# codeMonkey339/Congestion-control-with-BitTorren

Hardware: AMD Instinct MI355X
Metric: GiB/s device-resident SHA-1 over 512KB chunks; % of HBM-read roofline (higher is better)
Workload: dtype u32; 1 GPU; 4096 x 524288 B chunks per GPU, device-resident (BASELINE config 2); chunks_per_gpu=4096, chunk_bytes=524288, kernel=split_u4_2prod, kernel_requested=auto, streams=1, parallelism=chunk-sharded x1, no collective

## Files before the change

### congestion-control-with-bittorren_amd/csrc/rt_device.hip

```cpp
#include <algorithm>
#include <cctype>
#include <cstdarg>
#include <cstdio>
#include <cstdlib>
#include <cstring>
#include <mutex>
#include <sched.h>
#include <string>
#include <vector>

#include "sha1_runtime_internal.h"

using namespace s1rt;

namespace {
std::string sysfs_line(const char* path) {
    char buf[4096] = {0};
    if (FILE* f = fopen(path, "r")) {
        if (!fgets(buf, sizeof buf, f)) buf[0] = 0;
        fclose(f);
    }
    return buf;
}

// ... 107 lines not shown
    va_end(ap);
    t_err = buf;
    return code;
}

std::string g_probe_err;
Device* g_dev = nullptr;

int device_count() {
    std::call_once(g_once, probe);
    return g_count;
}

int ensure_slots(Device& D, int n) {
    for (int i = 0; i < n && i < kMaxSlots; ++i) {
        Slot& s = D.slot[i];
        if (s.stream) continue;
        HIP_TRY(hipEventCreateWithFlags(&s.done, hipEventDisableTiming));
        HIP_TRY(hipEventCreateWithFlags(&s.copied, hipEventDisableTiming));
        HIP_TRY(hipStreamCreateWithFlags(&s.stream, hipStreamNonBlocking));
    }
    return SHA1CHUNK_OK;
}

int ensure_copy(Device& D) {
    if (!D.copy) HIP_TRY(hipStreamCreateWithFlags(&D.copy, hipStreamNonBlocking));
    return SHA1CHUNK_OK;
}

int get_device(Device** out) {
    if (device_count() <= 0) return fail(SHA1CHUNK_ENODEV, "%s", g_probe_err.c_str());
    if (t_dev < 0 || t_dev >= g_count) return fail(SHA1CHUNK_EINVAL, "bad device %d", t_dev);
    Device& D = g_dev[t_dev];
    HIP_TRY(hipSetDevice(D.id));
    if (!D.ready.load(std::memory_order_acquire)) {
        std::lock_guard<std::mutex> lk(D.mu);
        if (!D.ready.load(std::memory_order_relaxed)) {
            hipDeviceProp_t pr;
            HIP_TRY(hipGetDeviceProperties(&pr, D.id));
            D.cus = pr.multiProcessorCount;
            int rc = ensure_slots(D, 1);
            if (rc) return rc;
            D.ready.store(true, std::memory_order_release);
        }
    }
    *out = &D;
    return SHA1CHUNK_OK;
}

int copies_issued(Slot& s, hipStream_t cs) {
    if (cs == s.stream) return SHA1CHUNK_OK;
    HIP_TRY(hipEventRecord(s.copied, cs));
    HIP_TRY(hipStreamWaitEvent(s.stream, s.copied, 0));
    return SHA1CHUNK_OK;
}

int discard_in_flight(Device& D) {
    for (auto& s : D.slot) {
        if (!s.busy) continue;
        s.busy = false;
        HIP_TRY(hipEventSynchronize(s.done));
    }
    return SHA1CHUNK_OK;
}

int drain_cus_take(Device* D) {
    const int want = static_cast<int>(
        std::max<uint64_t>(1, std::min<uint64_t>({static_cast<uint64_t>(D->cus), 1024, env_u64("SHA1CHUNK_VQ_CUS", 64)})));
    const int budget = static_cast<int>(std::min<uint64_t>(
        static_cast<uint64_t>(D->cus), env_u64("SHA1CHUNK_VQ_CU_BUDGET", static_cast<uint64_t>(D->cus / 2))));
    std::lock_guard<std::mutex> lk(D->drain_mu);
    const int left = budget - D->drain_cus;
    const int take = std::min(want, left);
    if (take < std::min(want, 8)) return 0;
    D->drain_cus += take;
    return take;
}

void drain_cus_give(int dev, int cus) {
    if (dev < 0 || dev >= g_count) return;
    std::lock_guard<std::mutex> lk(g_dev[dev].drain_mu);
    g_dev[dev].drain_cus -= cus;
}
}

extern "C" {

int s1be_device_count(void) {
    const int n = device_count();
    if (n <= 0) fail(SHA1CHUNK_ENODEV, "%s", g_probe_err.c_str());
    return n;
}

int s1be_set_device(int device) {
    const int n = device_count();
    if (n <= 0) return fail(SHA1CHUNK_ENODEV, "%s", g_probe_err.c_str());
    if (device < 0 || device >= n) return fail(SHA1CHUNK_EINVAL, "device %d of %d", device, n);
    t_dev = device;
    return SHA1CHUNK_OK;
}

const char* s1be_last_error(void) { return t_err.c_str(); }

int s1be_device_pci_bus_id(int device, char* buf, size_t len) {
    const int n = device_count();
    if (n <= 0) return fail(SHA1CHUNK_ENODEV, "%s", g_probe_err.c_str());
    if (device < 0 || device >= n) return fail(SHA1CHUNK_EINVAL, "device %d of %d", device, n);
    if (len > static_cast<size_t>(INT32_MAX)) len = INT32_MAX;
    HIP_TRY(hipDeviceGetPCIBusId(buf, static_cast<int>(len), g_dev[device].id));
    return SHA1CHUNK_OK;
}

int s1be_receive_cpus(int device, unsigned slot, void* mask, size_t len, unsigned* domains) {
    const int n = device_count();
    if (n <= 0) return fail(SHA1CHUNK_ENODEV, "%s", g_probe_err.c_str());
    if (device < 0 || device >= n) return fail(SHA1CHUNK_EINVAL, "device %d of %d", device, n);
    const std::vector<cpu_set_t>& dom = receive_domains(g_dev[device].id);
    if (dom.empty()) return fail(SHA1CHUNK_EINVAL, "no CPU of this process's affinity mask found");
    const cpu_set_t& d = dom[slot % dom.size()];
    memset(mask, 0, len);
    memcpy(mask, &d, sizeof d);
    if (domains) *domains = static_cast<unsigned>(dom.size());
    return CPU_COUNT(&d);
}

}
```

### congestion-control-with-bittorren_amd/csrc/sha1_kernels.h

```cpp
#pragma once

#include <hip/hip_runtime.h>
#include <stdint.h>

struct BatchArgs {
    const uint8_t* base;
    const uint64_t* off;
    const uint32_t* len;
    uint32_t ulen;
    uint32_t n;
    const uint32_t* order;
    uint8_t* dig;
    const uint32_t* init_state;
    uint64_t prefix_bytes;
    uint32_t* out_state;
    const uint32_t* plan;
};

hipError_t launch_lane(const BatchArgs& A, hipStream_t st);
hipError_t launch_fused(const BatchArgs& A, hipStream_t st);
bool split_unit_built(int unit_blocks);
hipError_t launch_split(const BatchArgs& A, int unit_blocks, hipStream_t st);
bool split_unit_study_built(int unit_blocks);
hipError_t launch_split_study(const BatchArgs& A, int unit_blocks, hipStream_t st);
uint32_t mixed_grid(uint32_t groups, int cus, uint32_t* hcap);
constexpr uint32_t kBigExact = 4096;
struct BigFix {
    const uint32_t* cnt;
    uint32_t tiles;
    const uint32_t* len;
    const uint32_t* id;
    uint32_t* order;
    uint32_t* sorted_len;
};
hipError_t launch_mixed(const BatchArgs& A, const uint32_t* sorted_len, const BigFix* big, uint32_t* plan, int cus,
                        const int* forced, hipStream_t st);
hipError_t launch_plan_layout(const BatchArgs& A, const uint32_t* sorted_len, const BigFix* big, uint32_t* plan,
                              hipStream_t st);
struct VqDrainArgs {
    const uint8_t* data;
    const uint64_t* off;
    const uint32_t* len;
    const uint8_t* exp;
    const uint32_t* grp;
    const uint32_t* pub;
    const uint32_t* stop;
    uint8_t* alive;
    uint8_t* res;
    uint32_t* done;
    uint32_t* last_done;
    uint8_t* dig;
    uint32_t* claim;
    uint32_t grp_ring;
    uint32_t pad;
    uint64_t idle_ticks;
    uint64_t life_ticks;
};
hipError_t launch_vq_drain(const VqDrainArgs& Q, uint32_t grid, hipStream_t st);

struct PvEntry {
    uint32_t session;
    uint32_t from;
    uint32_t upto;
    uint32_t len;
    uint32_t final;
    uint32_t gen;
    uint32_t pad[2];
};
struct PvArgs {
    const uint8_t* data;
    uint64_t stride;
    const PvEntry* work;
    uint32_t n;
    uint32_t sessions;
    uint32_t* state;
    const uint32_t* expected;
    uint32_t* result;
    uint32_t* done;
    const uint8_t* dummy;
};
hipError_t launch_progress(const PvArgs& P, int depth, hipStream_t st);
hipError_t launch_progress_shared(const PvArgs& P, hipStream_t st);

struct UpdateArgs {
    uint8_t* ctx;
    uint64_t n_contexts;
    const uint32_t* index;
    uint32_t n;
    const uint8_t* base;
    const uint64_t* off;
    const uint32_t* len;
    uint64_t* mid_off;
    uint32_t* mid_len;
    uint32_t* state;
    uint8_t* dig;
};
hipError_t launch_update_init(const UpdateArgs& U, hipStream_t st);
hipError_t launch_update_pre(const UpdateArgs& U, hipStream_t st);
hipError_t launch_update_post(const UpdateArgs& U, hipStream_t st);
hipError_t launch_update_final(const UpdateArgs& U, hipStream_t st);

struct GatherArgs {
    const uint8_t* base;
// ... 33 lines not shown
```

### congestion-control-with-bittorren_amd/csrc/sha1_kernels.hip

```cpp
#include <hip/hip_runtime.h>
#include <stdint.h>

#include <algorithm>
#include <cstdlib>
#include <cstring>

#include "sha1_split.hpp"

#define PLAN_SPLIT4 0.743
#define PLAN_SPLIT8 0.860
#define PLAN_FUSED4T 1.254
#define PLAN_FUSED4S 1.334
#define PLAN_FUSED8T 2.502
#define PLAN_FUSED8S 2.628
#define PLAN_FUSED_SHARE 0.955

__global__ __launch_bounds__(256) void sha1_lane_kernel(BatchArgs A) {
    const uint32_t e = blockIdx.x * blockDim.x + threadIdx.x;
    if (e >= A.n) return;
    const Entry en = fetch_entry(A, e);
    uint32_t h[5];
    load_init(A, en.id, h);
    lane_blocks(A, en, 0, h);
    emit(A, en.id, h);
// ... 777 lines not shown
    if (t < kMaxCand) {
        uint64_t key = t < nref ? (uint64_t)__float_as_uint(cmk[t]) << 32 | t : ~0ull;
#pragma unroll
        for (uint32_t m = 32; m >= 1; m >>= 1) key = min(key, (uint64_t)__shfl_xor(key, m));
        if (lane == 0u) red[wv] = key;
    }
    __syncthreads();
    if (t == 0) {
        ts[5] = __builtin_amdgcn_s_memrealtime();
        cs[5] = __builtin_amdgcn_s_memtime();
        uint64_t key = red[0];
#pragma unroll
        for (uint32_t w = 1; w < kMaxCand / 64; ++w) key = min(key, red[w]);
        uint32_t bi = (uint32_t)key;
        if (cmk[2] <= cmk[bi] * 1.005f) bi = 2;
        plan[0] = cmode[bi];
        plan[1] = cmode[bi] == 1 ? 0u : chead[bi];
        plan[2] = cmode[bi] == 1 ? 0u : cf[bi];
#pragma unroll
        for (int i = 1; i < 6; ++i) plan[7 + i] = static_cast<uint32_t>(ts[i] - ts[0]);
#pragma unroll
        for (int i = 1; i < 6; ++i) plan[13 + i] = static_cast<uint32_t>(cs[i] - cs[0]);
#pragma unroll
        for (int i = 0; i < 3; ++i) plan[20 + i] = static_cast<uint32_t>(sub[i] - cs[0]);
        plan[23] = nrun;
#pragma unroll
        for (int i = 0; i < 3; ++i) plan[24 + i] = static_cast<uint32_t>(bsub[i] - cs[0]);
        plan[27] = simcyc;
    }
}

__device__ __forceinline__ uint64_t splitmix64(uint64_t x) {
    uint64_t z = x + 0x9E3779B97F4A7C15ull;
    z = (z ^ (z >> 30)) * 0xBF58476D1CE4E5B9ull;
    z = (z ^ (z >> 27)) * 0x94D049BB133111EBull;
    return z ^ (z >> 31);
}

__global__ __launch_bounds__(kSynthThreads) void synth_fill_kernel(uint8_t* dst, const uint64_t* off,
                                                         const uint32_t* lens, uint32_t ulen,
                                                         uint64_t first, uint64_t seed) {
    const uint64_t c = blockIdx.x;
    const uint32_t len = lens ? lens[c] : ulen;
    uint8_t* out = dst + (off ? off[c] : c * (uint64_t)ulen);
    const uint64_t key = seed ^ ((first + c) << 24);
    const uint32_t nw = len >> 3;
    uint64_t* o = reinterpret_cast<uint64_t*>(out);
    for (uint32_t w = threadIdx.x; w < nw; w += blockDim.x) o[w] = splitmix64(key ^ (uint64_t)w);
    const uint32_t rem = len & 7u;
    if (rem && threadIdx.x == 0) {
        const uint64_t v = splitmix64(key ^ (uint64_t)nw);
        for (uint32_t b = 0; b < rem; ++b) out[8ull * nw + b] = (uint8_t)(v >> (8 * b));
    }
}

__global__ __launch_bounds__(256) void compare_kernel(const uint8_t* dig, const uint8_t* exp,
                                                      uint32_t n, uint8_t* mismatch) {
    const uint32_t i = blockIdx.x * blockDim.x + threadIdx.x;
    if (i >= n) return;
    uint32_t diff = 0;
#pragma unroll
    for (int b = 0; b < 20; ++b) diff |= (uint32_t)(dig[20ull * i + b] ^ exp[20ull * i + b]);
    mismatch[i] = diff ? 1 : 0;
}

hipError_t launch_lane(const BatchArgs& A, hipStream_t st) {
    if (A.n == 0) return hipSuccess;
    const uint32_t grid = (A.n + 255u) / 256u;
    hipLaunchKernelGGL(sha1_lane_kernel, dim3(grid), dim3(256), 0, st, A);
    return hipGetLastError();
}

hipError_t launch_fused(const BatchArgs& A, hipStream_t st) {
    if (A.n == 0) return hipSuccess;
    hipLaunchKernelGGL(sha1_fused_kernel, dim3((A.n + 255u) / 256u), dim3(256), 0, st, A);
    return hipGetLastError();
}

__attribute__((weak)) bool split_unit_study_built(int) { return false; }
__attribute__((weak)) hipError_t launch_split_study(const BatchArgs&, int, hipStream_t) {
    return hipErrorInvalidValue;
}

bool split_unit_built(int u) { return u == 1 || u == 4 || u == 11 || split_unit_study_built(u); }

hipError_t launch_split(const BatchArgs& A, int unit_blocks, hipStream_t st) {
    if (A.n == 0) return hipSuccess;
    const uint32_t groups = (A.n + 63u) / 64u;
    switch (unit_blocks) {
    case 1: hipLaunchKernelGGL((sha1_split_kernel<1, 1>), dim3(groups), dim3(128), 0, st, A); break;
    case 4:
        hipLaunchKernelGGL((sha1_split_kernel<4, 1, kSplitV<4>, kSplitNProd<4>>), dim3(groups),
                           dim3(64 * (1 + kSplitNProd<4>) + ((kSplitV<4> & kVSkipWave2) ? 64 : 0)), 0,
                           st, A);
        break;
    case 11:
        if (A.off == nullptr && A.order == nullptr)
            hipLaunchKernelGGL((sha1_split_kernel<2, 2, kSplit8V & ~kVCoop, 2>), dim3((groups + 1) / 2), dim3(512),
                               0, st, A);
        else
            hipLaunchKernelGGL((sha1_split_kernel<2, 2, kSplit8V, 2>), dim3((groups + 1) / 2), dim3(512), 0,
                               st, A);
        break;
    default: return launch_split_study(A, unit_blocks, st);
    }
    return hipGetLastError();
}

uint32_t mixed_grid(uint32_t groups, int cus, uint32_t* hcap) {
    *hcap = std::min<uint32_t>(std::min<uint32_t>(groups, 4u * (uint32_t)cus), kPlanMaxH);
    return groups;
}

hipError_t launch_plan_layout(const BatchArgs& A, const uint32_t* sorted_len, const BigFix* big, uint32_t* plan,
                              hipStream_t st) {
    if (A.n == 0) return hipSuccess;
    const uint32_t groups = (A.n + 63u) / 64u;
    const uint32_t words = (groups + 31u) / 32u;
    uint64_t* lay_tb = reinterpret_cast<uint64_t*>(plan + 64);
    uint32_t* lay_bits = reinterpret_cast<uint32_t*>(lay_tb + words);
    uint32_t* lay_blk = lay_bits + words;
    hipLaunchKernelGGL(plan_layout_kernel, dim3(words), dim3(kLayoutThreads), 0, st, A, sorted_len,
                       big ? *big : BigFix{}, lay_tb, lay_bits, lay_blk);
    return hipGetLastError();
}

hipError_t launch_mixed(const BatchArgs& A, const uint32_t* sorted_len, const BigFix* big, uint32_t* plan, int cus,
                        const int* forced, hipStream_t st) {
    if (A.n == 0) return hipSuccess;
    const uint32_t groups = (A.n + 63u) / 64u;
    uint32_t hcap;
    const uint32_t grid = mixed_grid(groups, cus, &hcap);
    const uint32_t words = (groups + 31u) / 32u;
    uint64_t* lay_tb = reinterpret_cast<uint64_t*>(plan + 64);
    uint32_t* lay_bits = reinterpret_cast<uint32_t*>(lay_tb + words);
    const uint32_t* lay_blk = lay_bits + words;
    if (!forced) {
        const hipError_t le = launch_plan_layout(A, sorted_len, big, plan, st);
        if (le != hipSuccess) return le;
    }
    hipLaunchKernelGGL(plan_mixed_kernel, dim3(1), dim3(kPlanThreads), 0, st, A, sorted_len,
                       (uint32_t)cus, hcap, forced ? 1 : 0, forced ? (uint32_t)forced[0] : 0u,
                       forced ? (uint32_t)forced[1] : 0u, forced ? (uint32_t)forced[2] : 0u, plan, lay_tb,
                       lay_bits, lay_blk);
    hipError_t e = hipGetLastError();
    if (e != hipSuccess) return e;
    BatchArgs B = A;
    B.plan = plan;
    const char* disp = getenv("SHA1CHUNK_MIXED_DISPATCH");
    const bool persistent = !(disp && !strcmp(disp, "hw"));
    if (persistent)
        hipLaunchKernelGGL(sha1_mixed_persistent_kernel, dim3((uint32_t)cus), dim3(kMixedThreads), 0, st, B,
                           plan + 3);
    else
        hipLaunchKernelGGL(sha1_mixed_kernel, dim3(grid), dim3(kMixedThreads), 0, st, B);
    return hipGetLastError();
}

hipError_t launch_vq_drain(const VqDrainArgs& Q, uint32_t grid, hipStream_t st) {
    hipLaunchKernelGGL(sha1_vq_drain_kernel, dim3(grid), dim3(kMixedThreads), 0, st, Q);
    return hipGetLastError();
}

hipError_t launch_synth(uint8_t* dst, const uint64_t* off, const uint32_t* lens, uint32_t ulen,
                        uint64_t first, uint64_t count, uint64_t seed, hipStream_t st) {
    if (count == 0) return hipSuccess;
    if (count > kSynthMaxChunks) return hipErrorInvalidValue;
    hipLaunchKernelGGL(synth_fill_kernel, dim3((uint32_t)count), dim3(kSynthThreads), 0, st, dst, off, lens,
                       ulen, first, seed);
    return hipGetLastError();
}

hipError_t launch_compare(const uint8_t* dig, const uint8_t* exp, uint32_t n, uint8_t* mismatch,
                          hipStream_t st) {
    if (n == 0) return hipSuccess;
    hipLaunchKernelGGL(compare_kernel, dim3((n + 255u) / 256u), dim3(256), 0, st, dig, exp, n,
                       mismatch);
    return hipGetLastError();
}

#ifdef SHA1CHUNK_CHECKED
extern "C" __attribute__((visibility("default"))) long long s1be_checked_violations(int reset) {
    int cur = 0, nd = 0;
    if (hipGetDevice(&cur) != hipSuccess || hipGetDeviceCount(&nd) != hipSuccess) return -1;
    long long total = 0;
    for (int d = 0; d < nd; ++d) {
// ... 15 lines not shown
```

### congestion-control-with-bittorren_amd/csrc/sha1_runtime.hip

```cpp
#include <algorithm>
#include <cstdio>
#include <cstdlib>
#include <cstring>
#include <mutex>
#include <numeric>
#include <string>
#include <thread>
#include <vector>

#include "sha1_runtime_internal.h"

using namespace s1rt;

namespace {
int split_unit(size_t n, int cus) {
    if (const char* e = getenv("SHA1CHUNK_SPLIT_UNIT")) return atoi(e);
    const size_t groups = (n + 63) / 64;
    if (groups <= size_t(cus)) return 4;
    if (groups <= size_t(cus) * 2) return 11;
    return 1;
}

hipError_t launch(int kernel, const BatchArgs& A, int cus, hipStream_t st) {
    switch (kernel) {
    case SHA1CHUNK_KERNEL_LANE: return launch_lane(A, st);
    case SHA1CHUNK_KERNEL_FUSED: return launch_fused(A, st);
    case SHA1CHUNK_KERNEL_SPLIT: return launch_split(A, split_unit(A.n, cus), st);
    default: return hipErrorInvalidValue;
    }
}

int check_batch(const BatchArgs& A) {
    if (A.n > 0xffffffffu - 1024u)
        return fail(SHA1CHUNK_EINVAL, "batch of %u chunks: at most 2^32 - 1025 per call", A.n);
    if (A.n > 0 && (reinterpret_cast<uintptr_t>(A.dig) & 3u))
        return fail(SHA1CHUNK_EALIGN, "digest buffer must be 4-byte aligned");
    return SHA1CHUNK_OK;
}
}

namespace s1rt {
int choose_kernel(int kernel, size_t n, int cus) {
    if (kernel != SHA1CHUNK_KERNEL_AUTO) return kernel;
    if (const char* f = getenv("SHA1CHUNK_FORCE_KERNEL")) {
        if (!strcmp(f, "lane")) return SHA1CHUNK_KERNEL_LANE;
        if (!strcmp(f, "fused")) return SHA1CHUNK_KERNEL_FUSED;
        if (!strcmp(f, "split")) return SHA1CHUNK_KERNEL_SPLIT;
    }
    const size_t groups = (n + 63) / 64;
    return groups <= size_t(cus) * 2 ? SHA1CHUNK_KERNEL_SPLIT : SHA1CHUNK_KERNEL_FUSED;
}

int launch_checked(int kernel, const BatchArgs& A, hipStream_t st, int cus) {
    if (kernel < SHA1CHUNK_KERNEL_LANE || kernel > SHA1CHUNK_KERNEL_SPLIT)
        return fail(SHA1CHUNK_EINVAL, "unknown kernel id %d", kernel);
    if (int rc = check_batch(A)) return rc;
    if (kernel == SHA1CHUNK_KERNEL_SPLIT && !split_unit_built(split_unit(A.n, cus)))
        return fail(SHA1CHUNK_EINVAL, "split shape %d is not in this library (A/B shapes: `make ab`)",
                    split_unit(A.n, cus));
    hipError_t e = launch(kernel, A, cus, st);
    if (e != hipSuccess) return fail(SHA1CHUNK_EHIP, "kernel launch: %s", hipGetErrorString(e));
    return SHA1CHUNK_OK;
}

bool use_mixed(size_t n, int cus) {
    if (getenv("SHA1CHUNK_FORCE_KERNEL")) return false;
    const char* e = getenv("SHA1CHUNK_MIXED");
    if (e && !strcmp(e, "0")) return false;
    if (e && !strcmp(e, "all")) return true;
    return (n + 63) / 64 > size_t(cus);
}

int launch_mixed_checked(const BatchArgs& A, const uint32_t* sorted_len, const BigFix* big, uint32_t* plan, int cus,
                         hipStream_t st) {
    if (int rc = check_batch(A)) return rc;
    int forced[3] = {0, 0, 0};
    bool force = false;
    if (const char* e = getenv("SHA1CHUNK_MIXED_PLAN")) {
        uint32_t hcap;
        const uint32_t groups = (A.n + 63u) / 64u;
        (void)mixed_grid(groups, cus, &hcap);
        if (sscanf(e, "%d,%d,%d", &forced[0], &forced[1], &forced[2]) != 3 || forced[0] < 0 ||
            forced[0] > 1 ||
            (forced[0] == 0 && (forced[1] < 0 || ((uint32_t)forced[1] > hcap && (uint32_t)forced[1] != groups) ||
                                (forced[2] != 4 && forced[2] != 8))))
            return fail(SHA1CHUNK_EINVAL,
                        "SHA1CHUNK_MIXED_PLAN=%s: want 0,H,F (0 <= H <= %u or H = %u, F 4|8) or 1,0,0", e,
                        hcap, groups);
        force = true;
    }
    hipError_t e = launch_mixed(A, sorted_len, big, plan, cus, force ? forced : nullptr, st);
    if (e != hipSuccess) return fail(SHA1CHUNK_EHIP, "mixed kernel launch: %s", hipGetErrorString(e));
    if (const char* d = getenv("SHA1CHUNK_MIXED_DEBUG"); d && atoi(d)) {
        uint32_t p[28];
        HIP_TRY(hipMemcpyAsync(p, plan, sizeof p, hipMemcpyDeviceToHost, st));
        HIP_TRY(hipStreamSynchronize(st));
        fprintf(stderr, "sha1chunk mixed plan: n=%u groups=%u cus=%d mode=%u H=%u F=%u\n", A.n,
                (A.n + 63u) / 64u, cus, p[0], p[1], p[2]);
        if (!force && p[12])
// ... 472 lines not shown
```

### congestion-control-with-bittorren_amd/csrc/sha1_runtime_internal.h

```cpp
#pragma once

#include <hip/hip_runtime.h>

#include <algorithm>
#include <atomic>
#include <cstdint>
#include <cstdlib>
#include <ctime>
#include <memory>
#include <mutex>
#include <sched.h>
#include <string>
#include <vector>

#include "../../include/sha1chunk.h"
#include "part_pool.hpp"
#include "sha1_kernels.h"

extern "C" const char* s1be_last_error(void);

namespace s1rt {
using s1host::PartPool;

int fail(int code, const char* fmt, ...) __attribute__((format(printf, 2, 3)));
// ... 13 lines not shown
    const char* e = getenv(name);
    return e ? strtoull(e, nullptr, 10) : dflt;
}

inline int64_t mono_ns() {
    timespec ts;
    clock_gettime(CLOCK_MONOTONIC, &ts);
    return int64_t(ts.tv_sec) * 1000000000 + ts.tv_nsec;
}

struct DevBuf {
    void* p = nullptr;
    size_t cap = 0;
    int ensure(size_t bytes) {
        if (bytes <= cap) return SHA1CHUNK_OK;
        if (p) (void)hipFree(p);
        p = nullptr;
        cap = 0;
        bytes = round_up(std::max(bytes, size_t(1) << 20), size_t(1) << 20);
        if (hipMalloc(&p, bytes) != hipSuccess)
            return fail(SHA1CHUNK_ENOMEM, "hipMalloc(%zu) failed", bytes);
        cap = bytes;
        return SHA1CHUNK_OK;
    }
};

struct PinBuf {
    void* p = nullptr;
    size_t cap = 0;
    int ensure(size_t bytes) {
        if (bytes <= cap) return SHA1CHUNK_OK;
        if (p) (void)hipHostFree(p);
        p = nullptr;
        cap = 0;
        bytes = round_up(std::max(bytes, size_t(1) << 20), size_t(1) << 20);
        if (hipHostMalloc(&p, bytes, hipHostMallocDefault) != hipSuccess)
            return fail(SHA1CHUNK_ENOMEM, "hipHostMalloc(%zu) failed", bytes);
        cap = bytes;
        return SHA1CHUNK_OK;
    }
};

constexpr int kMaxSlots = 8;

struct Slot {
    PinBuf hpin;
    PinBuf hdig;
    DevBuf dmem;
    DevBuf ddig;
    hipStream_t stream = nullptr;
    hipEvent_t done = nullptr;
    hipEvent_t copied = nullptr;
    bool busy = false;
    std::vector<uint32_t> ids;
};

struct Device {
    std::mutex mu;
    std::atomic<bool> ready{false};
    int id = -1;
    int cus = 256;
    Slot slot[kMaxSlots];
    hipStream_t copy = nullptr;
    DevBuf small;
    PinBuf small_pin;
    std::unique_ptr<PartPool> pack;
    std::mutex drain_mu;
    int drain_cus = 0;
};

extern Device* g_dev;
extern std::string g_probe_err;
extern thread_local int t_dev;
int device_count();
int get_device(Device** out);
int ensure_slots(Device& D, int n);
int ensure_copy(Device& D);
int copies_issued(Slot& s, hipStream_t cs);
int discard_in_flight(Device& D);
const cpu_set_t* near_cpus(int id);
const std::vector<cpu_set_t>& receive_domains(int id);
int drain_cus_take(Device* D);
void drain_cus_give(int dev, int cus);

int choose_kernel(int kernel, size_t n, int cus);
int launch_checked(int kernel, const BatchArgs& A, hipStream_t st, int cus = 256);
bool use_mixed(size_t n, int cus);
int launch_mixed_checked(const BatchArgs& A, const uint32_t* sorted_len, const BigFix* big, uint32_t* plan, int cus,
                         hipStream_t st);
bool host_pinned(const void* p);
int pack_threads();

int vq_copy_helpers();
unsigned ring_flags();
int vq_stream_create(hipStream_t* s);
}
```

### congestion-control-with-bittorren_amd/csrc/sha1_split.hpp

```cpp
#ifndef SHA1_SPLIT_HPP
#define SHA1_SPLIT_HPP

#include <hip/hip_runtime.h>
#include <stdint.h>

#include "sha1_device.hpp"
#include "sha1_kernels.h"

using namespace s1;

namespace {

struct Entry {
    uint32_t id;
    const uint8_t* p;
    uint32_t len;
};

#ifdef SHA1CHUNK_CHECKED
__device__ unsigned int g_checked_oob;

__device__ __forceinline__ uint32_t checked_index(uint32_t i, uint32_t n, const char* what) {
    if (i < n) return i;
    if (atomicAdd(&g_checked_oob, 1u) < 8u)
// ... 400 lines not shown
        read_w_group<3>(slot, Wn);
        __builtin_amdgcn_sched_barrier(0);
        RoundsW<R + 40, 80, WK>::run(v, Wc);
    } else {
        constexpr int R = PH != 0 ? 10 : 0;
        if constexpr (jn == 0) split_barrier_or_timed<V>(bw);
        RoundsW<0, R, WK>::run(v, Wc);
        __builtin_amdgcn_sched_barrier(0);
        read_w_group<0>(slot, Wn);
        __builtin_amdgcn_sched_barrier(0);
        RoundsW<R, R + 20, WK>::run(v, Wc);
        __builtin_amdgcn_sched_barrier(0);
        read_w_group<1>(slot, Wn);
        __builtin_amdgcn_sched_barrier(0);
        RoundsW<R + 20, R + 40, WK>::run(v, Wc);
        __builtin_amdgcn_sched_barrier(0);
        read_w_group<2>(slot, Wn);
        __builtin_amdgcn_sched_barrier(0);
        RoundsW<R + 40, R + 60, WK>::run(v, Wc);
        __builtin_amdgcn_sched_barrier(0);
        read_w_group<3>(slot, Wn);
        __builtin_amdgcn_sched_barrier(0);
        RoundsW<R + 60, 80, WK>::run(v, Wc);
    }
    if constexpr (MASK) {
        const bool live = k < T;
#pragma unroll
        for (int i = 0; i < 5; ++i) h[i] = live ? h[i] + v[i] : h[i];
    } else {
#pragma unroll
        for (int i = 0; i < 5; ++i) h[i] += v[i];
    }
}

template <int U, int J, int V, bool MASK, int PH = 0>
struct ConsumeUnits {
    __device__ __forceinline__ static void run(uint32_t k0, uint32_t T, uint32_t (&h)[5],
                                               uint32_t (&Wa)[80], uint32_t (&Wb)[80],
                                               const uint8_t* ring, int lane, uint64_t& bw) {
        if constexpr (J < 2 * U) {
            consume_block<U, J, V, MASK, PH>(k0 + J, T, h, Wa, Wb, ring, lane, bw);
            ConsumeUnits<U, J + 1, V, MASK, PH>::run(k0, T, h, Wb, Wa, ring, lane, bw);
        }
    }
};

template <int U, int V, int PH>
__device__ __forceinline__ void consume_all(const BatchArgs& A, const Entry& en, bool valid, uint32_t T,
                                            uint32_t units, const uint8_t* ring, int lane) {
    uint32_t h[5];
    load_init(A, en.id, h);
    uint32_t Wa[80], Wb[80];
    split_barrier();
    read_w_group<0>(ring + lane * 16, Wa);
    read_w_group<1>(ring + lane * 16, Wa);
    read_w_group<2>(ring + lane * 16, Wa);
    read_w_group<3>(ring + lane * 16, Wa);
    const uint32_t Tmin = __builtin_amdgcn_readfirstlane(wave_min(valid ? T : 0xffffffffu));
    const uint32_t full = (V & kVUnmask) ? min(Tmin, units * U) / (2 * U) * (2 * U) : 0u;
    uint32_t k = 0;
    uint64_t bw = 0;
    const uint64_t t0 = (V & kVProbe) ? __builtin_amdgcn_s_memtime() : 0;
    for (; k < full; k += 2 * U) {
        ConsumeUnits<U, 0, V, false, PH>::run(k, T, h, Wa, Wb, ring, lane, bw);
    }
    for (; k < units * U; k += 2 * U) {
        ConsumeUnits<U, 0, V, true, PH>::run(k, T, h, Wa, Wb, ring, lane, bw);
    }
    if constexpr ((V & kVProbe) != 0) {
        const uint64_t tot = __builtin_amdgcn_s_memtime() - t0;
        if (lane == 0) {
            uint32_t* o = reinterpret_cast<uint32_t*>(A.dig + 20ull * (en.id & ~63u));
            o[0] = (uint32_t)bw;
            o[1] = (uint32_t)(bw >> 32);
            o[2] = (uint32_t)tot;
            o[3] = (uint32_t)(tot >> 32);
            o[4] = units * U;
        }
        return;
    }
    if (valid) emit(A, en.id, h);
}

template <int U, int PAIRS, int V, int NPROD>
__device__ __forceinline__ void split_body(const BatchArgs& A, uint8_t* lds, uint32_t wg) {
    constexpr bool WK = (V & kVWK) != 0;
    static_assert(PAIRS * 2 * U * kWBlockBytes <= 160 * 1024, "LDS");
    static_assert(NPROD == 1 || (PAIRS == 1 && (U == 2 * NPROD || U == NPROD)) ||
                      (PAIRS == 2 && U == NPROD && (V & kVLayout8) != 0),
                  "two producers: one stage (U = 4) or one block (U = 2, 8-wave layout) each per unit");
    int wave = __builtin_amdgcn_readfirstlane(threadIdx.x >> 6);
    if constexpr ((V & kVSimdRole) != 0) {
        static_assert(PAIRS == 1 && NPROD == 2 && U == 2, "SIMD roles: one pair, two producers, 2-block units");
        uint32_t* slots = reinterpret_cast<uint32_t*>(lds);
        const uint32_t hw = __builtin_amdgcn_s_getreg((31u << 11) | (0u << 6) | 4u);
        if ((threadIdx.x & 63u) == 0) slots[1 + wave] = (hw >> 4) & 3u;
        if (threadIdx.x == 0) slots[0] = cu_turn(hw);
        __syncthreads();
        const uint32_t cs = (__builtin_amdgcn_readfirstlane(slots[0]) & 1u) ? 2u : 0u;
        int wc = -1, wi = -1;
        for (int w = 0; w < 4; ++w)
            if (wc < 0 && slots[1 + w] == cs) wc = w;
        if (wc < 0) wc = 0;
        for (int w = 0; w < 4; ++w)
            if (wi < 0 && w != wc && slots[1 + w] == (cs ^ 2u)) wi = w;
        if (wi < 0) wi = wc == 3 ? 2 : 3;
        int rank = 0;
        for (int w = 0; w < wave; ++w) rank += (w != wc && w != wi) ? 1 : 0;
        __syncthreads();
        if (wave == wi) return;
        wave = wave == wc ? 0 : 1 + rank;
    }
    if constexpr ((V & kVSkipWave2) != 0) {
        static_assert(NPROD == 2 && PAIRS == 1, "skip-wave layout is for two producers");
        if (wave == 2) return;
        if (wave > 2) wave -= 1;
    }
    int pair = wave % PAIRS;
    bool producer = wave >= PAIRS;
    uint32_t pidx = producer ? (uint32_t)(wave - PAIRS) / PAIRS : 0u;
    if constexpr ((V & kVLayout8) != 0) {
        static_assert(PAIRS == 2 && NPROD == 2, "8-wave layout: two pairs, two producers each");
        if (wave == 4 || wave == 6) return;
        producer = (wave & 1) != 0;
        pair = producer ? (((wave >> 1) & 1) ^ ((V & kVCross) ? 1 : 0)) : (wave >> 1);
        pidx = producer ? (uint32_t)(wave >> 2) : 0u;
    }
    const int lane = threadIdx.x & 63;
    uint8_t* ring = lds + pair * (2 * U * kWBlockBytes);
    const uint32_t group = wg * PAIRS + (uint32_t)pair;
    const uint32_t e = group * 64u + (uint32_t)lane;
    const bool valid = e < A.n;
    Entry en = fetch_entry(A, valid ? e : fallback_entry(A, group));
    if (!valid) en.len = 0;
    const uint32_t T = valid ? (A.out_state ? (en.len >> 6) : total_blocks(en.len)) : 0u;
    uint32_t Tmax = __builtin_amdgcn_readfirstlane(wave_max(T));
    if constexpr (PAIRS > 1) {
        uint32_t* slots = reinterpret_cast<uint32_t*>(lds);
        if (!producer && lane == 0) slots[pair] = Tmax;
        __syncthreads();
#pragma unroll
        for (int q = 0; q < PAIRS; ++q) Tmax = max(Tmax, slots[q]);
        Tmax = __builtin_amdgcn_readfirstlane(Tmax);
        __syncthreads();
    }
    const uint32_t units = (Tmax + 2 * U - 1) / (2 * U) * 2;

    if (producer) {
        const uint32_t S = bulk_stages(en, valid);
        if constexpr (U == NPROD) {
            const uint32_t K = S * 2u;
            uint32_t B0[16], B1[16];
            uint32_t k = pidx;
            uint64_t pbw = 0;
            uint64_t* const pb = (V & kVProbe) ? &pbw : nullptr;
            const uint64_t pt0 = (V & kVProbe) ? __builtin_amdgcn_s_memtime() : 0;
            if constexpr ((V & kVCoop) != 0) {
                const u32x4u* src[4];
                coop_sources<4>(A, group, (uint32_t)lane, src);
                if (pidx < K) coop4_load(src, pidx, B0);
                if (pidx + NPROD < K) coop4_load(src, pidx + NPROD, B1);
                for (; k + NPROD < K; k += 2 * NPROD) {
                    produce_own_block_coop<U, WK, NPROD>(src, k, K, B0, ring, (uint32_t)lane, pb);
                    produce_own_block_coop<U, WK, NPROD>(src, k + NPROD, K, B1, ring, (uint32_t)lane, pb);
                }
                if (k < K) {
                    produce_own_block_coop<U, WK, NPROD>(src, k, K, B0, ring, (uint32_t)lane, pb);
                    k += NPROD;
// ... 7 lines not shown
                }
                if (k < K) {
                    produce_own_block<U, WK, NPROD>(en, k, K, B0, ring, lane, pb);
                    k += NPROD;
                }
            }
            for (; k < units * U; k += NPROD) {
                uint32_t w[16];
                if (k < T) tail_block_words(en, k, w);
                produce_block<U, WK, NPROD>(k, w, ring, lane, pb);
            }
            if constexpr ((V & kVProbe) != 0) {
                const uint64_t tot = __builtin_amdgcn_s_memtime() - pt0;
                if (lane == 0) {
                    uint32_t* o = reinterpret_cast<uint32_t*>(A.dig + 20ull * (group * 64u + 1u + pidx));
                    o[0] = (uint32_t)pbw;
                    o[1] = (uint32_t)(pbw >> 32);
                    o[2] = (uint32_t)tot;
                    o[3] = (uint32_t)(tot >> 32);
                    o[4] = units * U;
                }
            }
            split_barrier();
            return;
        }
        uint32_t s = pidx;
        if constexpr ((V & kVCoop) != 0) {
            const u32x4u* src[8];
            coop_sources<8>(A, group, (uint32_t)lane, src);
            uint32_t C0[32], C1[32];
            if (pidx < S) coop_load(src, pidx, C0);
            if (pidx + NPROD < S) coop_load(src, pidx + NPROD, C1);
            for (; s + NPROD < S; s += 2 * NPROD) {
                produce_stage_coop<U, WK, NPROD>(src, s, S, C0, ring, (uint32_t)lane);
                produce_stage_coop<U, WK, NPROD>(src, s + NPROD, S, C1, ring, (uint32_t)lane);
            }
            if (s < S) {
                produce_stage_coop<U, WK, NPROD>(src, s, S, C0, ring, (uint32_t)lane);
                s += NPROD;
            }
        } else {
            Stage A0, A1;
            if (pidx < S) load_stage(en.p + 128ull * pidx, A0);
            if (pidx + NPROD < S) load_stage(en.p + 128ull * (pidx + NPROD), A1);
            for (; s + NPROD < S; s += 2 * NPROD) {
                produce_stage<U, WK, NPROD>(en, s, S, A0, ring, lane);
                produce_stage<U, WK, NPROD>(en, s + NPROD, S, A1, ring, lane);
            }
            if (s < S) {
                produce_stage<U, WK, NPROD>(en, s, S, A0, ring, lane);
                s += NPROD;
            }
        }
        for (; 2 * s < units * U; s += NPROD) {
#pragma unroll
            for (int half = 0; half < 2; ++half) {
                const uint32_t k = 2 * s + half;
                uint32_t w[16];
                if (k < T) tail_block_words(en, k, w);
                produce_block<U, WK, NPROD>(k, w, ring, lane);
            }
        }
        split_barrier();
    } else {
        if constexpr ((V & kVPhase2) != 0) {
            if (pair == 1)
                consume_all<U, V, 3>(A, en, valid, T, units, ring, lane);
            else
                consume_all<U, V, 1>(A, en, valid, T, units, ring, lane);
            return;
        }
        if constexpr ((V & kVPhase) != 0) {
            if (pair == 1) {
                consume_all<U, V, 2>(A, en, valid, T, units, ring, lane);
                return;
            }
        }
        consume_all<U, V, 0>(A, en, valid, T, units, ring, lane);
    }
}

constexpr int kSplit8V = kVWK | kVUnmask | kVLayout8 | kVCross | kVCoop;

template <int U, int PAIRS, int V = kSplitV<U>, int NPROD = 1>
__global__ __launch_bounds__((kSplitThreads<PAIRS, V, NPROD>)) void sha1_split_kernel(
    BatchArgs A) {
    __shared__ __attribute__((aligned(16))) uint8_t lds[PAIRS * 2 * U * kWBlockBytes];
    split_body<U, PAIRS, V, NPROD>(A, lds, blockIdx.x);
}


template <typename V>
__device__ __forceinline__ void fused_stage(uint32_t s, uint32_t S, const Entry& en, Stage& cur,
                                            uint32_t (&h)[5]) {
#pragma unroll
    for (int half = 0; half < 2; ++half) {
        uint32_t w[16];
#pragma unroll
        for (int j = 0; j < 16; ++j) w[j] = bswap_fresh(cur.w[16 * half + j]);
        if (half == 1 && s + 2 < S) load_stage<V>(en.p + 128ull * (s + 2), cur);
        compress(h, w);
    }
}

template <typename V>
__device__ __forceinline__ void fused_lane_stages_v(const Entry& en, uint32_t S, uint32_t (&h)[5]) {
    Stage A0, A1;
    if (S > 0) load_stage<V>(en.p, A0);
    if (S > 1) load_stage<V>(en.p + 128, A1);
    uint32_t s = 0;
    for (; s + 1 < S; s += 2) {
        fused_stage<V>(s, S, en, A0, h);
        fused_stage<V>(s + 1, S, en, A1, h);
    }
    if (s < S) fused_stage<V>(s, S, en, A0, h);
}

__device__ __forceinline__ void fused_stage_any(uint32_t s, uint32_t S, const Entry& en, RawSpan<32>& cur,
                                                uint32_t (&h)[5]) {
    const uint32_t sh = static_cast<uint32_t>(reinterpret_cast<uintptr_t>(en.p) & 3u);
    uint32_t w[16];
    shift_raw<32, 0, 16>(cur, sh, w);
#pragma unroll
    for (int j = 0; j < 16; ++j) w[j] = bswap_fresh(w[j]);
    compress(h, w);
    shift_raw<32, 16, 16>(cur, sh, w);
#pragma unroll
    for (int j = 0; j < 16; ++j) w[j] = bswap_fresh(w[j]);
    if (s + 2 < S) load_raw<32>(en.p + 128ull * (s + 2), cur);
    compress(h, w);
}

__device__ __forceinline__ void fused_lane_stages_any(const Entry& en, uint32_t S, uint32_t (&h)[5]) {
    RawSpan<32> A0, A1;
    if (S > 0) load_raw<32>(en.p, A0);
    if (S > 1) load_raw<32>(en.p + 128, A1);
    uint32_t s = 0;
    for (; s + 1 < S; s += 2) {
        fused_stage_any(s, S, en, A0, h);
        fused_stage_any(s + 1, S, en, A1, h);
    }
    if (s < S) fused_stage_any(s, S, en, A0, h);
}

__device__ __forceinline__ void fused_lane_stages(const Entry& en, bool valid, uint32_t S, uint32_t (&h)[5]) {
    if (wave_all(!valid || (reinterpret_cast<uintptr_t>(en.p) & 15u) == 0))
        fused_lane_stages_v<uint4>(en, S, h);
    else
        fused_lane_stages_any(en, S, h);
}

__device__ __forceinline__ void fused_body(const BatchArgs& A, uint32_t e) {
    const uint32_t group = e / 64u;
    const bool valid = e < A.n;
    Entry en = fetch_entry(A, valid ? e : fallback_entry(A, group));
    if (!valid) en.len = 0;
    uint32_t h[5];
    load_init(A, en.id, h);
    const uint32_t S = bulk_stages(en, valid);
    fused_lane_stages(en, valid, S, h);
    if (valid) {
        lane_blocks(A, en, 2u * S, h);
        emit(A, en.id, h);
    }
}


__device__ __forceinline__ void coop_compress(const uint32_t (&cur)[32], uint32_t (&h)[5]) {
#pragma unroll
    for (int half = 0; half < 2; ++half) {
// ... 92 lines not shown
```

Measured before the change: 332.1 GiB/s.

## Add quad-lane split SHA-1 kernel spreading 16 chunks per workgroup across CUs

Adds a new split producer/consumer kernel shape in which four lanes cooperate on one chunk. Message words are broadcast with DPP quad moves, and the two producer waves write W+K schedules into a 5 KiB-per-block LDS ring. The runtime picks it when the 16-chunk workgroup count fits in the CUs not held by drain work. The aim is to use many more CUs for mid-sized batches than the 64-chunks-per-group shape does. The cost is more redundant round work per lane, fewer digests per wave, and a new heuristic that reads the drain CU budget under a mutex.

```diff
diff --git a/congestion-control-with-bittorren_amd/csrc/rt_device.hip b/congestion-control-with-bittorren_amd/csrc/rt_device.hip
--- a/congestion-control-with-bittorren_amd/csrc/rt_device.hip
+++ b/congestion-control-with-bittorren_amd/csrc/rt_device.hip
@@ -213,6 +213,12 @@
     std::lock_guard<std::mutex> lk(g_dev[dev].drain_mu);
     g_dev[dev].drain_cus -= cus;
 }
+
+int drain_cus_held() {
+    if (!g_dev || t_dev < 0 || t_dev >= g_count) return 0;
+    std::lock_guard<std::mutex> lk(g_dev[t_dev].drain_mu);
+    return g_dev[t_dev].drain_cus;
+}
 }
 
 extern "C" {
diff --git a/congestion-control-with-bittorren_amd/csrc/sha1_kernels.h b/congestion-control-with-bittorren_amd/csrc/sha1_kernels.h
--- a/congestion-control-with-bittorren_amd/csrc/sha1_kernels.h
+++ b/congestion-control-with-bittorren_amd/csrc/sha1_kernels.h
@@ -19,6 +19,7 @@
 
 hipError_t launch_lane(const BatchArgs& A, hipStream_t st);
 hipError_t launch_fused(const BatchArgs& A, hipStream_t st);
+constexpr int kSplitUnitQuad = 416;
 bool split_unit_built(int unit_blocks);
 hipError_t launch_split(const BatchArgs& A, int unit_blocks, hipStream_t st);
 bool split_unit_study_built(int unit_blocks);
diff --git a/congestion-control-with-bittorren_amd/csrc/sha1_kernels.hip b/congestion-control-with-bittorren_amd/csrc/sha1_kernels.hip
--- a/congestion-control-with-bittorren_amd/csrc/sha1_kernels.hip
+++ b/congestion-control-with-bittorren_amd/csrc/sha1_kernels.hip
@@ -883,7 +883,9 @@
     return hipErrorInvalidValue;
 }
 
-bool split_unit_built(int u) { return u == 1 || u == 4 || u == 11 || split_unit_study_built(u); }
+bool split_unit_built(int u) {
+    return u == 1 || u == 4 || u == 11 || u == kSplitUnitQuad || split_unit_study_built(u);
+}
 
 hipError_t launch_split(const BatchArgs& A, int unit_blocks, hipStream_t st) {
     if (A.n == 0) return hipSuccess;
@@ -903,6 +905,9 @@
             hipLaunchKernelGGL((sha1_split_kernel<2, 2, kSplit8V, 2>), dim3((groups + 1) / 2), dim3(512), 0,
                                st, A);
         break;
+    case kSplitUnitQuad:
+        hipLaunchKernelGGL((sha1_split_kernel<4, 1, kSplitQuadV, 2>), dim3((A.n + 15u) / 16u), dim3(256), 0, st, A);
+        break;
     default: return launch_split_study(A, unit_blocks, st);
     }
     return hipGetLastError();
diff --git a/congestion-control-with-bittorren_amd/csrc/sha1_runtime.hip b/congestion-control-with-bittorren_amd/csrc/sha1_runtime.hip
--- a/congestion-control-with-bittorren_amd/csrc/sha1_runtime.hip
+++ b/congestion-control-with-bittorren_amd/csrc/sha1_runtime.hip
@@ -15,6 +15,7 @@
 namespace {
 int split_unit(size_t n, int cus) {
     if (const char* e = getenv("SHA1CHUNK_SPLIT_UNIT")) return atoi(e);
+    if ((n + 15) / 16 <= size_t(std::max(0, cus - drain_cus_held()))) return kSplitUnitQuad;
     const size_t groups = (n + 63) / 64;
     if (groups <= size_t(cus)) return 4;
     if (groups <= size_t(cus) * 2) return 11;
diff --git a/congestion-control-with-bittorren_amd/csrc/sha1_runtime_internal.h b/congestion-control-with-bittorren_amd/csrc/sha1_runtime_internal.h
--- a/congestion-control-with-bittorren_amd/csrc/sha1_runtime_internal.h
+++ b/congestion-control-with-bittorren_amd/csrc/sha1_runtime_internal.h
@@ -119,6 +119,7 @@
 const std::vector<cpu_set_t>& receive_domains(int id);
 int drain_cus_take(Device* D);
 void drain_cus_give(int dev, int cus);
+int drain_cus_held();
 
 int choose_kernel(int kernel, size_t n, int cus);
 int launch_checked(int kernel, const BatchArgs& A, hipStream_t st, int cus = 256);
diff --git a/congestion-control-with-bittorren_amd/csrc/sha1_split.hpp b/congestion-control-with-bittorren_amd/csrc/sha1_split.hpp
--- a/congestion-control-with-bittorren_amd/csrc/sha1_split.hpp
+++ b/congestion-control-with-bittorren_amd/csrc/sha1_split.hpp
@@ -506,8 +506,230 @@
     if (valid) emit(A, en.id, h);
 }
 
+constexpr int kVQuad = 8192 * 4;
+constexpr int kQuadBlockBytes = 5 * 1024;
+constexpr int kQuadWaitRound = 4;
+constexpr int kSplitQuadV = kVWK | kVUnmask | kVSkipWave2 | kVCoop | kVQuad;
+
+template <int SEL>
+__device__ __forceinline__ uint32_t quad_bcast(uint32_t x) {
+    return (uint32_t)__builtin_amdgcn_update_dpp(0, (int)x, SEL * 0x55, 0xf, 0xf, true);
+}
+
+template <int T, int END>
+struct RoundsQ {
+    __device__ __forceinline__ static void run(uint32_t (&v)[5], const uint32_t (&W)[20]) {
+        if constexpr (T < END) {
+            round_step<T, true>(v, quad_bcast<(T >> 2) & 3>(W[4 * (T >> 4) + (T & 3)]));
+            RoundsQ<T + 1, END>::run(v, W);
+        }
+    }
+};
+
+__device__ __forceinline__ void quad_read_w(const uint8_t* slot, uint32_t (&W)[20]) {
+#pragma unroll
+    for (int q = 0; q < 5; ++q) {
+        const uint4 x = *reinterpret_cast<const uint4*>(slot + q * 1024);
+        W[4 * q + 0] = x.x;
+        W[4 * q + 1] = x.y;
+        W[4 * q + 2] = x.z;
+        W[4 * q + 3] = x.w;
+    }
+}
+
+template <int U, int J, int V, bool MASK>
+__device__ __forceinline__ void quad_consume_block(uint32_t k, uint32_t T, uint32_t (&h)[5],
+                                                   const uint32_t (&Wc)[20], uint32_t (&Wn)[20],
+                                                   const uint8_t* ring, int lane, uint64_t& bw) {
+    constexpr int jn = (J + 1) % U;
+    constexpr int slot_idx = (((J + 1) / U) & 1) * U + jn;
+    const uint8_t* slot = ring + slot_idx * kQuadBlockBytes + lane * 16;
+    uint32_t v[5] = {h[0], h[1], h[2], h[3], h[4]};
+    if constexpr (jn == 0) split_barrier_or_timed<V>(bw);
+    __builtin_amdgcn_sched_barrier(0);
+    quad_read_w(slot, Wn);
+    __builtin_amdgcn_sched_barrier(0);
+    RoundsQ<0, kQuadWaitRound>::run(v, Wc);
+    __builtin_amdgcn_sched_barrier(0);
+    __builtin_amdgcn_s_waitcnt(0xC07F);
+    __builtin_amdgcn_sched_barrier(0);
+    RoundsQ<kQuadWaitRound, 80>::run(v, Wc);
+    if constexpr (MASK) {
+        const bool live = k < T;
+#pragma unroll
+        for (int i = 0; i < 5; ++i) h[i] = live ? h[i] + v[i] : h[i];
+    } else {
+#pragma unroll
+        for (int i = 0; i < 5; ++i) h[i] += v[i];
+    }
+}
+
+template <int U, int J, int V, bool MASK>
+struct QuadConsumeUnits {
+    __device__ __forceinline__ static void run(uint32_t k0, uint32_t T, uint32_t (&h)[5], uint32_t (&Wa)[20],
+                                               uint32_t (&Wb)[20], const uint8_t* ring, int lane, uint64_t& bw) {
+        if constexpr (J < 2 * U) {
+            quad_consume_block<U, J, V, MASK>(k0 + J, T, h, Wa, Wb, ring, lane, bw);
+            QuadConsumeUnits<U, J + 1, V, MASK>::run(k0, T, h, Wb, Wa, ring, lane, bw);
+        }
+    }
+};
+
+template <int T>
+struct QuadSchedWrite {
+    __device__ __forceinline__ static void run(uint32_t (&w)[16], uint8_t* slot, bool j1, bool j2,
+                                               const uint32_t (&kq)[5]) {
+        if constexpr (T < 80) {
+            if constexpr (T >= 16) sched_step<T>(w);
+            if constexpr ((T & 15) == 15) {
+                constexpr int q = T >> 4;
+                uint32_t o[4];
+#pragma unroll
+                for (int i = 0; i < 4; ++i) {
+                    const uint32_t lo = j1 ? w[4 + i] : w[i], hi = j1 ? w[12 + i] : w[8 + i];
+                    o[i] = (j2 ? hi : lo) + kq[q];
+                }
+                *reinterpret_cast<uint4*>(slot + q * 1024) = make_uint4(o[0], o[1], o[2], o[3]);
+            }
+            QuadSchedWrite<T + 1>::run(w, slot, j1, j2, kq);
+        }
+    }
+};
+
+template <int U>
+__device__ __forceinline__ void quad_produce_block(uint32_t k, uint32_t (&w)[16], uint8_t* ring, int lane,
+                                                   const uint32_t (&kq)[5]) {
+    const uint32_t m = k / U, j = k - m * U;
+    QuadSchedWrite<0>::run(w, ring + ((m & 1u) * U + j) * kQuadBlockBytes + lane * 16, (lane & 1) != 0,
+                           (lane & 2) != 0, kq);
+    if ((k & 1u) == 1u) split_barrier();
+}
+
+__device__ __forceinline__ void quad_block_words(const uint32_t (&x)[4], uint32_t (&w)[16]) {
+    uint32_t y[4];
+#pragma unroll
+    for (int i = 0; i < 4; ++i) y[i] = bswap(x[i]);
+#pragma unroll
+    for (int i = 0; i < 4; ++i) {
+        w[i] = quad_bcast<0>(y[i]);
+        w[4 + i] = quad_bcast<1>(y[i]);
+        w[8 + i] = quad_bcast<2>(y[i]);
+        w[12 + i] = quad_bcast<3>(y[i]);
+    }
+}
+
+__device__ __forceinline__ void quad_load_stage(const u32x4u* src, uint32_t s, uint32_t (&x)[8]) {
+#pragma unroll
+    for (int b = 0; b < 2; ++b) {
+        const u32x4u v = src[8u * s + 4u * b];
+        x[4 * b + 0] = v.x;
+        x[4 * b + 1] = v.y;
+        x[4 * b + 2] = v.z;
+        x[4 * b + 3] = v.w;
+    }
+}
+
+template <int U>
+__device__ __forceinline__ void quad_produce_stage(const u32x4u* src, uint32_t s, uint32_t S, uint32_t (&cur)[8],
+                                                   uint8_t* ring, int lane, const uint32_t (&kq)[5]) {
+    uint32_t x0[4] = {cur[0], cur[1], cur[2], cur[3]}, x1[4] = {cur[4], cur[5], cur[6], cur[7]};
+    if (s + 4 < S) quad_load_stage(src, s + 4, cur);
+    uint32_t w[16];
+    quad_block_words(x0, w);
+    quad_produce_block<U>(2 * s, w, ring, lane, kq);
+    quad_block_words(x1, w);
+    quad_produce_block<U>(2 * s + 1, w, ring, lane, kq);
+}
+
+template <int U, int V>
+__device__ __forceinline__ void quad_consume_all(const BatchArgs& A, const Entry& en, bool valid, uint32_t T,
+                                                 uint32_t units, const uint8_t* ring, int lane, uint32_t wg) {
+    uint32_t h[5];
+    load_init(A, en.id, h);
+    uint32_t Wa[20], Wb[20];
+    split_barrier();
+    quad_read_w(ring + lane * 16, Wa);
+    const uint32_t Tmin = __builtin_amdgcn_readfirstlane(wave_min(valid ? T : 0xffffffffu));
+    const uint32_t full = min(Tmin, units * U) / (2 * U) * (2 * U);
+    uint32_t k = 0;
+    uint64_t bw = 0;
+    const uint64_t t0 = (V & kVProbe) ? __builtin_amdgcn_s_memtime() : 0;
+    for (; k < full; k += 2 * U) QuadConsumeUnits<U, 0, V, false>::run(k, T, h, Wa, Wb, ring, lane, bw);
+    for (; k < units * U; k += 2 * U) QuadConsumeUnits<U, 0, V, true>::run(k, T, h, Wa, Wb, ring, lane, bw);
+    if constexpr ((V & kVProbe) != 0) {
+        const uint64_t tot = __builtin_amdgcn_s_memtime() - t0;
+        if (lane == 0) {
+            uint32_t* o = reinterpret_cast<uint32_t*>(A.dig + 20ull * (wg * 16u));
+            o[0] = (uint32_t)bw;
+            o[1] = (uint32_t)(bw >> 32);
+            o[2] = (uint32_t)tot;
+            o[3] = (uint32_t)(tot >> 32);
+            o[4] = units * U;
+        }
+        return;
+    }
+    if (valid && (lane & 3) == 0) emit(A, en.id, h);
+}
+
+template <int U, int V, int NPROD>
+__device__ __forceinline__ void quad_split_body(const BatchArgs& A, uint8_t* ring, uint32_t wg) {
+    static_assert(U == 4 && NPROD == 2 && (V & kVSkipWave2) != 0 && (V & kVWK) != 0 && (V & kVUnmask) != 0,
+                  "quad shape: 4-block units, two producers on waves 1 and 3, W+K shipped");
+    int wave = __builtin_amdgcn_readfirstlane(threadIdx.x >> 6);
+    if (wave == 2) return;
+    const bool producer = wave != 0;
+    const uint32_t pidx = wave == 3 ? 1u : 0u;
+    const int lane = threadIdx.x & 63;
+    const uint32_t e = wg * 16u + ((uint32_t)lane >> 2);
+    const bool valid = e < A.n;
+    Entry en = fetch_entry(A, valid ? e : min(wg * 16u, A.n - 1u));
+    if (!valid) en.len = 0;
+    const uint32_t T = valid ? (A.out_state ? (en.len >> 6) : total_blocks(en.len)) : 0u;
+    const uint32_t Tmax = __builtin_amdgcn_readfirstlane(wave_max(T));
+    const uint32_t units = (Tmax + 2 * U - 1) / (2 * U) * 2;
+    if (!producer) {
+        quad_consume_all<U, V>(A, en, valid, T, units, ring, lane, wg);
+        return;
+    }
+    uint32_t kq[5];
+#pragma unroll
+    for (int q = 0; q < 5; ++q) {
+        const uint32_t t = 16u * q + 4u * ((uint32_t)lane & 3u);
+        kq[q] = t < 20 ? K0 : t < 40 ? K1 : t < 60 ? K2 : K3;
+    }
+    const uint32_t S = bulk_stages(en, valid);
+    const u32x4u* src = reinterpret_cast<const u32x4u*>(en.p) + (lane & 3);
+    uint32_t C0[8], C1[8];
+    uint32_t s = pidx;
+    if (s < S) quad_load_stage(src, s, C0);
+    if (s + 2 < S) quad_load_stage(src, s + 2, C1);
+    for (; s + 2 < S; s += 4) {
+        quad_produce_stage<U>(src, s, S, C0, ring, lane, kq);
+        quad_produce_stage<U>(src, s + 2, S, C1, ring, lane, kq);
+    }
+    if (s < S) {
+        quad_produce_stage<U>(src, s, S, C0, ring, lane, kq);
+        s += 2;
+    }
+    for (; 2 * s < units * U; s += 2) {
+#pragma unroll
+        for (int half = 0; half < 2; ++half) {
+            const uint32_t k = 2 * s + half;
+            uint32_t w[16];
+            if (k < T) tail_block_words(en, k, w);
+            quad_produce_block<U>(k, w, ring, lane, kq);
+        }
+    }
+    split_barrier();
+}
+
 template <int U, int PAIRS, int V, int NPROD>
 __device__ __forceinline__ void split_body(const BatchArgs& A, uint8_t* lds, uint32_t wg) {
+    if constexpr ((V & kVQuad) != 0) {
+        static_assert(PAIRS == 1, "quad shape: one consumer per workgroup");
+        quad_split_body<U, V, NPROD>(A, lds, wg);
+        return;
+    }
     constexpr bool WK = (V & kVWK) != 0;
     static_assert(PAIRS * 2 * U * kWBlockBytes <= 160 * 1024, "LDS");
     static_assert(NPROD == 1 || (PAIRS == 1 && (U == 2 * NPROD || U == NPROD)) ||
@@ -681,10 +903,13 @@
 
 constexpr int kSplit8V = kVWK | kVUnmask | kVLayout8 | kVCross | kVCoop;
 
+template <int U, int PAIRS, int V>
+constexpr int kSplitLdsBytes = (V & kVQuad) ? 2 * U * kQuadBlockBytes : PAIRS * 2 * U * kWBlockBytes;
+
 template <int U, int PAIRS, int V = kSplitV<U>, int NPROD = 1>
 __global__ __launch_bounds__((kSplitThreads<PAIRS, V, NPROD>)) void sha1_split_kernel(
     BatchArgs A) {
-    __shared__ __attribute__((aligned(16))) uint8_t lds[PAIRS * 2 * U * kWBlockBytes];
+    __shared__ __attribute__((aligned(16))) uint8_t lds[kSplitLdsBytes<U, PAIRS, V>];
     split_body<U, PAIRS, V, NPROD>(A, lds, blockIdx.x);
 }
 
```

Measured after the change: 341.6 GiB/s (median of 6 runs). +2.8%, better.
